# sparsemat/sprs

Measured on AMD Instinct MI355X. Metric: CSR SpMV GFLOP/s, higher is better.
Workload: dtype f64; 1 GPU; R-MAT 10M x 10M, ~32 nnz/row (Graph500 a,b,c,d=.57,.19,.19,.05; seed 1); rows=10000000, cols=10000000, nnz=321592231, index_bytes=8, indptr_bytes=8, partition=single GPU, first_spmv_plan=nnz tiles

## Files before the change

### sprs_amd/csrc/spmv_band_kernels.hpp

```cpp
#pragma once
#include "spmv_shared.hpp"

namespace sprs_hip {
namespace {

typedef uint32_t u32x4 __attribute__((ext_vector_type(4)));

constexpr int WT = 512;
constexpr int WPASS = WT / (WAVE * 2);
constexpr int EPL = WT / WAVE;
constexpr int HOT_THREADS = 1024;
constexpr int HOT_WAVES = HOT_THREADS / WAVE;
constexpr int CNT = 256;
constexpr uint32_t ROW_START = 0x8000u;
constexpr uint32_t ROW_START32 = 0x80000000u;
static_assert(WPASS == 4 && EPL == 8, "wave tile geometry");

struct BandPiece {
    const uint32_t *rowidx;
    const uint32_t *tile_row;
    double *out;
    uint64_t ent0;
    uint64_t nnz;
    uint32_t nr, ntiles;
    uint32_t x0;
    uint32_t to_y;
    uint32_t range0;
    uint32_t pad;
};

struct Seg {
    uint32_t piece, tile0, ntiles, range0, run, pad0, pad1, pad2;
};

struct alignas(64) HotSeg {
    uint64_t ent0, nnz;
    const uint32_t *tile_row;
    uint64_t out_off;
    uint32_t x0, tile0, ntiles, range0;
    uint32_t run, pad0, pad1, pad2;
};
static_assert(sizeof(HotSeg) == 64, "one scalar load");

struct ColdGroup {
    uint32_t first_block, first_piece, npieces;
};

#ifdef SPRS_HIP_EMU
#define SPRS_GLOBAL_AS
#define SPRS_HOT_WAVES_ATTR
#else
#define SPRS_GLOBAL_AS __attribute__((address_space(1)))
#define SPRS_HOT_WAVES_ATTR __attribute__((amdgpu_waves_per_eu(5, 5)))
#endif
struct PieceView {
    const SPRS_GLOBAL_AS uint32_t *rowidx, *tile_row;
    SPRS_GLOBAL_AS double *out;
    uint64_t ent0, nnz;
    uint32_t nr, ntiles, x0, to_y, range0;
    __device__ __forceinline__ PieceView(const BandPiece &p)
        : rowidx((const SPRS_GLOBAL_AS uint32_t *)p.rowidx), tile_row((const SPRS_GLOBAL_AS uint32_t *)p.tile_row),
          out((SPRS_GLOBAL_AS double *)p.out), ent0(p.ent0), nnz(p.nnz), nr(p.nr), ntiles(p.ntiles), x0(p.x0), to_y(p.to_y),
          range0(p.range0) {}
};

__device__ __forceinline__ uint32_t band_scan_incl_u32(uint32_t v, uint32_t lane) {
    (void)lane;
    int x = (int)v;
    x += __builtin_amdgcn_update_dpp(0, x, 0x111, 0xf, 0xf, true);
    x += __builtin_amdgcn_update_dpp(0, x, 0x112, 0xf, 0xf, true);
    x += __builtin_amdgcn_update_dpp(0, x, 0x114, 0xf, 0xf, true);
    x += __builtin_amdgcn_update_dpp(0, x, 0x118, 0xf, 0xf, true);
    x += __builtin_amdgcn_update_dpp(0, x, 0x142, 0xa, 0xf, false);
    x += __builtin_amdgcn_update_dpp(0, x, 0x143, 0xc, 0xf, false);
    return (uint32_t)x;
}

template <int CTRL, int ROW_MASK, bool BOUND>
__device__ __forceinline__ void band_seg_step(double &S, uint32_t &F) {
    const int lo = __builtin_amdgcn_update_dpp(0, __double2loint(S), CTRL, ROW_MASK, 0xf, BOUND);
    const int hi = __builtin_amdgcn_update_dpp(0, __double2hiint(S), CTRL, ROW_MASK, 0xf, BOUND);
    const uint32_t fs = (uint32_t)__builtin_amdgcn_update_dpp(0, (int)F, CTRL, ROW_MASK, 0xf, BOUND);
    const double vs = __hiloint2double(hi, lo);
    S = F ? S : vs + S;
    F |= fs;
}

__device__ __forceinline__ void band_seg_scan(double &S, uint32_t &F, uint32_t lane) {
    (void)lane;
    band_seg_step<0x111, 0xf, true>(S, F);
    band_seg_step<0x112, 0xf, true>(S, F);
    band_seg_step<0x114, 0xf, true>(S, F);
    band_seg_step<0x118, 0xf, true>(S, F);
    band_seg_step<0x142, 0xa, false>(S, F);
    band_seg_step<0x143, 0xc, false>(S, F);
}

__device__ __forceinline__ double band_lane_below(double S, uint32_t lane) {
    (void)lane;
    const int lo = __builtin_amdgcn_update_dpp(0, __double2loint(S), 0x138, 0xf, 0xf, true);
    const int hi = __builtin_amdgcn_update_dpp(0, __double2hiint(S), 0x138, 0xf, 0xf, true);
    return __hiloint2double(hi, lo);
}

__device__ __forceinline__ double band_read_lane63(double v) {
    const int lo = __builtin_amdgcn_readlane(__double2loint(v), WAVE - 1);
    const int hi = __builtin_amdgcn_readlane(__double2hiint(v), WAVE - 1);
    return __hiloint2double(hi, lo);
}

__device__ __forceinline__ void wave_lds_fence() {
    __builtin_amdgcn_fence(__ATOMIC_RELEASE, "wavefront");
    __builtin_amdgcn_wave_barrier();
    __builtin_amdgcn_fence(__ATOMIC_ACQUIRE, "wavefront");
}

constexpr int STG = 128;
constexpr uint32_t hot_lds_bytes(uint32_t xt_log2) { return ((1u << xt_log2) + (uint32_t)HOT_WAVES * 128u) * 8u; }

struct Pending {
    uint32_t cnt = 0;
    uint32_t row0 = 0;
    bool first_to_carry = false;
};

template <typename Out>
__device__ __forceinline__ void band_flush(Pending &pd, uint32_t lane, SPRS_GLOBAL_AS double *carry, const double *stage, Out out) {
    for (uint32_t j = lane; j < pd.cnt; j += WAVE) {
        const double v = stage[j];
        if (j == 0 && pd.first_to_carry) *carry = v;
        else out(pd.row0 + j, v);
    }
    wave_lds_fence();
    pd.cnt = 0;
}

template <bool DEFER, typename Out>
__device__ __forceinline__ void band_tile_sums(const double (&pr)[EPL], uint32_t fb, uint32_t lane, uint32_t R0, double &open, bool &mine,
                                               uint32_t &last, SPRS_GLOBAL_AS double *carry, double *stage, Pending &pd, Out out) {
    const uint32_t nfl = (uint32_t)__popc(fb);
    const uint32_t incl = band_scan_incl_u32(nfl, lane);
    const uint32_t prefix = incl - nfl;
    const uint32_t nf = (uint32_t)__builtin_amdgcn_readlane((int)incl, WAVE - 1);
    double ev[EPL];
    double run = 0.0, head = 0.0;
    uint32_t seen = 0;
#pragma unroll
    for (int q = 0; q < EPL; ++q) {
        ev[q] = run;
        if ((fb >> q) & 1u) {
            if (seen == 0) head = run;
            run = 0.0;
            ++seen;
        }
        run += pr[q];
    }
    double S = run;
    uint32_t F = seen ? 1u : 0u;
    band_seg_scan(S, F, lane);
    double before = band_lane_below(S, lane);
    if (prefix == 0) before = open + before;
    const double vhead = before + head;
    for (uint32_t lo = 0; lo < nf; lo += STG) {
#pragma unroll
        for (int q = 0; q < EPL; ++q) {
            if ((fb >> q) & 1u) {
                const uint32_t below = fb & ((1u << q) - 1u);
                const uint32_t o = prefix + (uint32_t)__popc(below) - lo;
                if (o < (uint32_t)STG) stage[o] = below ? ev[q] : vhead;
            }
        }
        wave_lds_fence();
        pd.cnt = nf - lo < (uint32_t)STG ? nf - lo : (uint32_t)STG;
        pd.row0 = R0 - 1u + lo;
        pd.first_to_carry = lo == 0 && !mine;
        if (!DEFER || lo + STG < nf) band_flush(pd, lane, carry, stage, out);
    }
    const double s63 = band_read_lane63(S);
    open = nf ? s63 : open + s63;
    if (nf) {
        mine = true;
        last = R0 + nf - 1;
    }
}

template <bool ACC, bool TOY>
__device__ __forceinline__ void band_cold_wave(const PieceView d, uint32_t r, uint32_t ct, const double *__restrict__ vals,
                                               const uint32_t *__restrict__ cid, const double *__restrict__ xp, double *__restrict__ y,
                                               double *__restrict__ carry, double *stage, uint32_t lane);

template <int XT_LOG2>
__global__ __launch_bounds__(HOT_THREADS) SPRS_HOT_WAVES_ATTR void band_hot_kernel(const HotSeg *__restrict__ hsegs,
                                                               const HotSeg *__restrict__ wg_first, const double *__restrict__ vals,
                                                               const uint16_t *__restrict__ cid, const double *__restrict__ xp,
                                                               double *__restrict__ partial, double *__restrict__ carry, uint32_t dbg,
                                                               unsigned long long *__restrict__ prof, uint32_t xcd_shares) {
    constexpr int XT = 1 << XT_LOG2;
    if constexpr (DEVTOOLS) {
        if (prof && threadIdx.x == 0) prof[3 * blockIdx.x] = (unsigned long long)wall_clock64();
    }
#ifdef SPRS_HIP_EMU
    static double lds[XT + HOT_WAVES * STG];
#else
    extern __shared__ __attribute__((aligned(16))) double lds[];
#endif
    double *xs = lds;
    const uint32_t tid = threadIdx.x, lane = tid & (WAVE - 1), wave = tid / WAVE;
    double *stage = lds + XT + wave * STG;
    uint32_t share = blockIdx.x;
    if (xcd_shares) {
        const uint32_t nq = gridDim.x >> 3, rem = gridDim.x & 7u, k = blockIdx.x & 7u;
        share = k * nq + (k < rem ? k : rem) + (blockIdx.x >> 3);
    }
    HotSeg nxt = wg_first[share];
    const uint32_t s0 = nxt.pad0, s1 = nxt.pad1;
    for (uint32_t s = s0; s < s1; ++s) {
        const HotSeg seg = nxt;
        if (s + 1 < s1) nxt = hsegs[s + 1];
        struct {
            const SPRS_GLOBAL_AS uint32_t *tile_row;
            SPRS_GLOBAL_AS double *out;
            uint64_t ent0, nnz;
            uint32_t x0;
        } d{(const SPRS_GLOBAL_AS uint32_t *)seg.tile_row, (SPRS_GLOBAL_AS double *)(partial + seg.out_off), seg.ent0, seg.nnz, seg.x0};
        if (s != s0) __syncthreads();
        {
            const dbl2 *src = (const dbl2 *)(xp + d.x0);
            dbl2 v[XT / (2 * HOT_THREADS)];
#pragma unroll
            for (int q = 0; q < XT / (2 * HOT_THREADS); ++q) v[q] = src[q * HOT_THREADS + tid];
#pragma unroll
            for (int q = 0; q < XT / (2 * HOT_THREADS); ++q) *(dbl2 *)&xs[2 * (q * HOT_THREADS + tid)] = v[q];
        }
        const uint32_t run = seg.run, n = seg.ntiles;
        dbl2 av[WPASS];
        u32x4 cw = {0u, 0u, 0u, 0u};
        uint32_t R0n = 0;
        auto request = [&](uint32_t w) {
            const uint64_t g = d.ent0 + (uint64_t)w * WT;
#pragma unroll
            for (int p = 0; p < WPASS; ++p) av[p] = __builtin_nontemporal_load((const dbl2 *)(vals + g + p * (WAVE * 2) + lane * 2));
            cw = __builtin_nontemporal_load((const u32x4 *)(cid + g + lane * EPL));
            R0n = d.tile_row[w];
        };
        uint32_t r = wave;
        uint32_t t = r * run;
        if (t < n) request(seg.tile0 + t);
        __syncthreads();
        if constexpr (DEVTOOLS) {
            if (prof && threadIdx.x == 0 && s == s0) prof[3 * blockIdx.x + 1] = (unsigned long long)wall_clock64();
        }
        double open = 0.0;
        bool mine = false;
        uint32_t last = 0;
        Pending pd;
        SPRS_GLOBAL_AS double *pd_slot = (SPRS_GLOBAL_AS double *)carry;
        while (t < n) {
            const uint32_t w = seg.tile0 + t;
            const uint64_t base = (uint64_t)w * WT;
            const uint32_t cnt = d.nnz - base < (uint64_t)WT ? (uint32_t)(d.nnz - base) : (uint32_t)WT;
            double pr[EPL], xv[EPL];
            uint32_t fb = 0;
#pragma unroll
            for (int p = 0; p < WPASS; ++p) {
                const uint32_t c2 = cw[p];
                xv[2 * p] = xs[c2 & (XT - 1)];
                xv[2 * p + 1] = xs[(c2 >> 16) & (XT - 1)];
                fb |= ((c2 >> 15) & 1u) << (2 * p);
                fb |= ((c2 >> 31) & 1u) << (2 * p + 1);
            }
#pragma unroll
            for (int p = 0; p < WPASS; ++p) {
                pr[2 * p] = av[p][0] * xv[2 * p];
                pr[2 * p + 1] = av[p][1] * xv[2 * p + 1];
            }
            if (cnt < (uint32_t)WT) {
#pragma unroll
                for (int q = 0; q < EPL; ++q) pr[q] = lane * EPL + q < cnt ? pr[q] : 0.0;
            }
            uint32_t R0 = R0n;
#ifndef SPRS_HIP_EMU
            asm volatile("" : "+v"(R0)::"memory");
#endif
            const uint32_t rend = (r + 1) * run < n ? (r + 1) * run : n;
            const bool range_ends = t + 1 >= rend;
            const uint32_t tn = range_ends ? (r + HOT_WAVES) * run : t + 1;
            SPRS_GLOBAL_AS double *cslot = (SPRS_GLOBAL_AS double *)carry + seg.range0 + r;
            auto out = [&](uint32_t row, double v) {
                if (DEVTOOLS && (dbg & 1u)) return;
                __builtin_nontemporal_store(v, &d.out[row]);

            };
            if (pd.cnt) band_flush(pd, lane, pd_slot, stage, out);
            if (tn < n) request(seg.tile0 + tn);
            if constexpr (DEVTOOLS) {
                if (dbg & 2u) fb &= 0x01u;
                if (dbg & 4u) fb = 0;
            }
            if (DEVTOOLS && (dbg & 8u)) {
                band_tile_sums<false>(pr, fb, lane, R0, open, mine, last, cslot, stage, pd, out);
            } else {
                band_tile_sums<true>(pr, fb, lane, R0, open, mine, last, cslot, stage, pd, out);
                pd_slot = cslot;
            }
            if (range_ends) {
                if (lane == 0) {
                    if (mine) d.out[last] = open;
                    else *cslot = open;
                }
                open = 0.0;
                mine = false;
                r += HOT_WAVES;
            }
            t = tn;
        }
        if (pd.cnt) band_flush(pd, lane, pd_slot, stage, [&](uint32_t row, double v) {
            if (DEVTOOLS && (dbg & 1u)) return;
            d.out[row] = v;
        });
    }
    if constexpr (DEVTOOLS) {
        if (prof) {
            __syncthreads();
            if (threadIdx.x == 0) prof[3 * blockIdx.x + 2] = (unsigned long long)wall_clock64();
        }
    }
}

struct ColdArgs {
    const BandPiece *pieces;
    const ColdGroup *groups;
    uint32_t ngroups;
    const double *vals;
    const uint32_t *cid;
    const double *xp;
    double *y, *carry;
    uint32_t block0, ct;
    uint32_t direct;
    BandPiece piece;
};

template <bool ACC, bool TOY>
__device__ __forceinline__ void band_cold_body(const ColdArgs &ca, uint32_t block, double (*stage_s)[STG]) {
    constexpr int WPB = CNT / WAVE;
    const BandPiece *__restrict__ pieces = ca.pieces;
    const ColdGroup *__restrict__ groups = ca.groups;
    const uint32_t ngroups = ca.ngroups, ct = ca.ct;
    const double *__restrict__ vals = ca.vals;
    const uint32_t *__restrict__ cid = ca.cid;
    const double *__restrict__ xp = ca.xp;
    double *__restrict__ y = ca.y;
    double *__restrict__ carry = ca.carry;
    const uint32_t tid = threadIdx.x, lane = tid & (WAVE - 1), wave = tid / WAVE;
    double *stage = stage_s[wave];
    const uint32_t bid = block + ca.block0;
    uint32_t r;
    BandPiece pc;
    if (ca.direct) {
        pc = ca.piece;
        r = block * WPB + wave;
    } else {
        uint32_t g = 0;
        while (g + 1 < ngroups && bid >= groups[g + 1].first_block) ++g;
        const ColdGroup cg = groups[g];
        const uint32_t lb = bid - cg.first_block;
        const uint32_t pi = cg.first_piece + (cg.npieces == 1 ? 0u : (lb & 7u));
        r = (cg.npieces == 1 ? lb : (lb >> 3)) * WPB + wave;
        pc = pieces[pi];
    }
    band_cold_wave<ACC, TOY>(PieceView(pc), r, ct, vals, cid, xp, y, carry, stage, lane);
}

template <bool ACC, bool TOY>
__device__ __forceinline__ void band_cold_wave(const PieceView d, uint32_t r, uint32_t ct, const double *__restrict__ vals,
                                               const uint32_t *__restrict__ cid, const double *__restrict__ xp, double *__restrict__ y,
                                               double *__restrict__ carry, double *stage, uint32_t lane) {
    const uint32_t t0 = r * ct;
    if (t0 >= d.ntiles) return;
    const uint32_t tend = t0 + ct < d.ntiles ? t0 + ct : d.ntiles;
    dbl2 av[WPASS];
    u32x4 lw[2];
    uint32_t R0n = 0;
    auto request = [&](uint32_t w) {
        const uint64_t gpos = d.ent0 + (uint64_t)w * WT;
#pragma unroll
        for (int p = 0; p < 2; ++p) lw[p] = __builtin_nontemporal_load((const u32x4 *)(cid + gpos + p * (WAVE * 4) + lane * 4));
#pragma unroll
        for (int p = 0; p < WPASS; ++p) av[p] = __builtin_nontemporal_load((const dbl2 *)(vals + gpos + p * (WAVE * 2) + lane * 2));
        R0n = d.tile_row[w];
    };
    request(t0);
    double open = 0.0;
    bool mine = false;
    uint32_t last = 0;
    SPRS_GLOBAL_AS double *cslot = (SPRS_GLOBAL_AS double *)carry + d.range0 + r;
    uint32_t yr_pre[4] = {0u, 0u, 0u, 0u}, yr_base = 0;
    auto emit_y = [&](uint32_t row, double v) {
        const uint32_t m = (row - yr_base) >> 6;
        uint32_t yr;
        if (TOY && m < 4u && ((row - yr_base) & 63u) == lane) yr = m == 0 ? yr_pre[0] : m == 1 ? yr_pre[1] : m == 2 ? yr_pre[2] : yr_pre[3];
        else yr = d.rowidx[row];
        if constexpr (ACC) y[yr] = y[yr] + v;
        else y[yr] = v;
    };
    auto emit_p = [&](uint32_t row, double v) { d.out[row] = v; };
    for (uint32_t w = t0; w < tend; ++w) {
        const uint64_t base = (uint64_t)w * WT;
        const uint32_t cnt = d.nnz - base < (uint64_t)WT ? (uint32_t)(d.nnz - base) : (uint32_t)WT;
        double xv[EPL];
        uint32_t fb = 0;
#pragma unroll
        for (int q = 0; q < EPL; ++q) {
            const uint32_t c = lw[q / 4][q % 4];
            xv[q] = xp[c & ~ROW_START32];
            fb |= (c >> 31) << q;
        }
        if constexpr (TOY) {
            yr_base = R0n - 1u;
#pragma unroll
            for (int m = 0; m < 4; ++m) {
                const uint32_t rr = yr_base + lane + 64u * (uint32_t)m;
                yr_pre[m] = d.rowidx[rr < d.nr ? rr : d.nr - 1u];
            }
        }
        double pr[EPL];
#pragma unroll
        for (int q = 0; q < EPL; ++q) pr[q] = av[q / 2][q % 2] * xv[q];
        if (cnt < (uint32_t)WT) {
#pragma unroll
            for (int q = 0; q < EPL; ++q) pr[q] = lane * EPL + q < cnt ? pr[q] : 0.0;
        }
        Pending pd;
        if constexpr (TOY) band_tile_sums<false>(pr, fb, lane, R0n, open, mine, last, cslot, stage, pd, emit_y);
        else band_tile_sums<false>(pr, fb, lane, R0n, open, mine, last, cslot, stage, pd, emit_p);
        if (w + 1 < tend) request(w + 1);
    }
    if (lane == 0) {
        if (!mine) *cslot = open;
        else if constexpr (TOY) emit_y(last, open);
        else emit_p(last, open);
    }
}

template <bool ACC, bool TOY>
__global__ __launch_bounds__(CNT, 8) void band_cold_kernel(ColdArgs ca) {
    __shared__ __attribute__((aligned(16))) double stage_s[CNT / WAVE][STG];
    band_cold_body<ACC, TOY>(ca, blockIdx.x, stage_s);
}

struct RangeRef {
    uint32_t piece, tile0;
    bool valid;
};

__device__ __forceinline__ RangeRef range_of(const Seg *__restrict__ segs, uint32_t nsegs, uint32_t i) {
    uint32_t lo = 0, hi = nsegs;
    while (hi - lo > 1) {
        const uint32_t mid = (lo + hi) >> 1;
        if (segs[mid].range0 <= i) lo = mid;
        else hi = mid;
    }
    const Seg sg = segs[lo];
    const uint32_t t = (i - sg.range0) * sg.run;
    return RangeRef{sg.piece, sg.tile0 + t, t < sg.ntiles};
}

__device__ __forceinline__ bool range_has_head(const BandPiece &d, uint32_t piece, uint32_t tile0, const uint16_t *__restrict__ cid_hot,
                                               const uint32_t *__restrict__ cid_cold, uint32_t nhot) {
    const uint64_t e = d.ent0 + (uint64_t)tile0 * WT;
    return piece < nhot ? !(cid_hot[e] & ROW_START) : !(cid_cold[e] & ROW_START32);
}

struct Spill {
    uint64_t dst;
    uint32_t first, n;
    uint32_t to_y, j;
};

struct RSpill {
    uint32_t j, first, n, pad;
};

__global__ __launch_bounds__(256) void bp_spill_kernel(const Seg *__restrict__ segs, uint32_t nsegs, uint32_t nranges,
                                                       const BandPiece *__restrict__ pieces, const uint64_t *__restrict__ pair_off,
                                                       uint32_t nhot, const uint16_t *__restrict__ cid_hot,
                                                       const uint32_t *__restrict__ cid_cold,
                                                       Spill *__restrict__ spills_y, Spill *__restrict__ spills_partial,
                                                       unsigned int *__restrict__ count) {
    const uint32_t i = blockIdx.x * blockDim.x + threadIdx.x;
    if (i >= nranges) return;
    const RangeRef rg = range_of(segs, nsegs, i);
    if (!rg.valid) return;
    const BandPiece d = pieces[rg.piece];
    if (!range_has_head(d, rg.piece, rg.tile0, cid_hot, cid_cold, nhot)) return;
    const uint32_t row = d.tile_row[rg.tile0] - 1;
    if (i > 0) {
        const RangeRef pj = range_of(segs, nsegs, i - 1);
        if (pj.valid && pj.piece == rg.piece && d.tile_row[pj.tile0] - 1 == row && range_has_head(d, pj.piece, pj.tile0, cid_hot, cid_cold, nhot))
            return;
    }
    uint32_t n = 1;
    for (uint32_t j = i + 1; j < nranges; ++j, ++n) {
        const RangeRef nj = range_of(segs, nsegs, j);
        if (!nj.valid || nj.piece != rg.piece || d.tile_row[nj.tile0] - 1 != row || !range_has_head(d, nj.piece, nj.tile0, cid_hot, cid_cold, nhot))
            break;
    }
    const bool first = d.to_y != 0;
    const unsigned int slot = atomicAdd(count + (first ? 0 : 1), 1u);
    (first ? spills_y : spills_partial)[slot] = Spill{d.to_y ? (uint64_t)d.rowidx[row] : pair_off[rg.piece] + row, i, n, d.to_y, d.rowidx[row]};
}

template <bool TO_Y>
__global__ __launch_bounds__(256) void band_carry_kernel(const Spill *__restrict__ spills, uint32_t nspills, const double *__restrict__ carry,
                                                         double *__restrict__ partial, double *__restrict__ y) {
    const uint32_t i = blockIdx.x * blockDim.x + threadIdx.x;
    if (i >= nspills) return;
    const Spill sp = spills[i];
    double *dst = (TO_Y ? y : partial) + sp.dst;
    double acc = *dst;
    for (uint32_t k = 0; k < sp.n; ++k) acc += carry[sp.first + k];
    *dst = acc;
}

template <bool CLEAR_Y>
__global__ __launch_bounds__(256) void band_gather_kernel(const double *__restrict__ x, const uint32_t *__restrict__ inv, uint32_t l0,
                                                          uint32_t l1, double *__restrict__ xp, double *__restrict__ y_zero, uint64_t rows) {
    const uint64_t t4 = ((uint64_t)blockIdx.x * blockDim.x + threadIdx.x) * 4;
    const uint64_t l = (uint64_t)l0 + t4;
    if (l + 4 <= (uint64_t)l1 && (l0 & 3u) == 0) {
        const u32x4 j = *(const u32x4 *)(inv + l);
        const double a0 = x[j[0]], a1 = x[j[1]], a2 = x[j[2]], a3 = x[j[3]];
        *(dbl2 *)(xp + l) = dbl2{a0, a1};
        *(dbl2 *)(xp + l + 2) = dbl2{a2, a3};
    } else {
        for (uint64_t q = l; q < (uint64_t)l1 && q < l + 4; ++q) xp[q] = x[inv[q]];
    }
    if (CLEAR_Y && y_zero) {
        if (t4 + 4 <= rows && ((uintptr_t)y_zero & 15) == 0) {
            *(dbl2 *)(y_zero + t4) = dbl2{0.0, 0.0};
            *(dbl2 *)(y_zero + t4 + 2) = dbl2{0.0, 0.0};
        } else {
            for (uint64_t r = t4; r < rows && r < t4 + 4; ++r) y_zero[r] = 0.0;
        }
    }
}

__global__ __launch_bounds__(256) void band_permute_kernel(const double *__restrict__ x, const uint32_t *__restrict__ perm,
                                                           uint64_t cols, double *__restrict__ xp, double *__restrict__ y_zero,
                                                           uint64_t rows, uint32_t first_label, uint32_t nref) {
    const uint64_t j = ((uint64_t)blockIdx.x * blockDim.x + threadIdx.x) * 4;
    const uint32_t span = nref - first_label;
    if (j + 4 <= cols && (((uintptr_t)x | (uintptr_t)perm) & 15) == 0) {
        const u32x4 l = *(const u32x4 *)(perm + j);
        const dbl2 a = *(const dbl2 *)(x + j), b = *(const dbl2 *)(x + j + 2);
        if (l[0] - first_label < span) xp[l[0]] = a[0];
        if (l[1] - first_label < span) xp[l[1]] = a[1];
        if (l[2] - first_label < span) xp[l[2]] = b[0];
        if (l[3] - first_label < span) xp[l[3]] = b[1];
    } else {
        for (uint64_t c = j; c < cols && c < j + 4; ++c) {
            const uint32_t l = perm[c];
            if (l - first_label < span) xp[l] = x[c];
        }
    }
    if (y_zero) {
        if (j + 4 <= rows && ((uintptr_t)y_zero & 15) == 0) {
            *(dbl2 *)(y_zero + j) = dbl2{0.0, 0.0};
            *(dbl2 *)(y_zero + j + 2) = dbl2{0.0, 0.0};
        } else {
            for (uint64_t r = j; r < rows && r < j + 4; ++r) y_zero[r] = 0.0;
        }
    }
}

constexpr int RU = 16;

__device__ __forceinline__ bool band_mask_bit(uint32_t m_lo, uint32_t m_hi, uint32_t lane) {
    (void)lane;
    return __builtin_amdgcn_inverse_ballot_w64(((unsigned long long)m_hi << 32) | m_lo);
}
__device__ __forceinline__ uint32_t band_mask_rank(uint32_t m_lo, uint32_t m_hi, uint32_t lane) {
    (void)lane;
    return __builtin_amdgcn_mbcnt_hi(m_hi, __builtin_amdgcn_mbcnt_lo(m_lo, 0u));
}

struct ReduceArgs {
    const double *partial;
    const unsigned long long *wmask;
    const uint32_t *wbase, *long_rows;
    const RSpill *rsp;
    const uint32_t *rsp_off;
    const double *carry;
    double *y;
    uint32_t n_long, np_pad, nwb;
};

template <bool ACC>
__device__ __forceinline__ void band_reduce_body(const ReduceArgs &ra, uint32_t block, uint32_t nblocks) {
    const double *__restrict__ partial = ra.partial;
    const unsigned long long *__restrict__ wmask = ra.wmask;
    const uint32_t *__restrict__ wbase = ra.wbase;
    const uint32_t *__restrict__ long_rows = ra.long_rows;
    double *__restrict__ y = ra.y;
    const uint32_t n_long = ra.n_long, np_pad = ra.np_pad, nwb = ra.nwb;
    const uint32_t lane = threadIdx.x & (WAVE - 1);
    const uint32_t wpb = blockDim.x / WAVE;
    const uint32_t xcd = block & 7u, inx = (block >> 3) * wpb + threadIdx.x / WAVE;
    const uint32_t per_xcd = (nwb + 7u) / 8u, waves_per_xcd = (nblocks >> 3) * wpb;
    for (uint32_t i = inx; i < per_xcd; i += waves_per_xcd) {
        const uint32_t wb = xcd * per_xcd + i;
        if (wb >= nwb) break;
        const uint64_t j = (uint64_t)wb * WAVE + lane;
        const uint64_t jc = j < n_long ? j : n_long - 1;
        const uint32_t r = long_rows[jc];
        uint32_t sb = 0, se = 0;
        if (ra.rsp_off) {
            sb = ra.rsp_off[wb];
            se = ra.rsp_off[wb + 1];
        }
        uint32_t h_jl = 0xFFFFFFFFu, h_first = 0, h_n = 0;
        double h_c = 0.0;
        if (sb + lane < se) {
            const RSpill rec = ra.rsp[sb + lane];
            h_jl = rec.j & (WAVE - 1);
            h_first = rec.first;
            h_n = rec.n;
            h_c = ra.carry[h_first];
        }
        double s = 0.0;
        const unsigned long long *mrow = wmask + (uint64_t)wb * np_pad;
        const uint32_t *brow = wbase + (uint64_t)wb * np_pad;
        unsigned long long mk_n = lane < np_pad ? mrow[lane] : 0ull;
        uint32_t bs_n = lane < np_pad ? brow[lane] : 0u;
        for (uint32_t k0 = 0; k0 < np_pad; k0 += WAVE) {
            const unsigned long long mk = mk_n;
            const uint32_t bs = bs_n;
            if (k0 + WAVE < np_pad) {
                const bool in = k0 + WAVE + lane < np_pad;
                mk_n = in ? mrow[k0 + WAVE + lane] : 0ull;
                bs_n = in ? brow[k0 + WAVE + lane] : 0u;
            }
            const uint32_t mk_lo = (uint32_t)mk, mk_hi = (uint32_t)(mk >> 32);
#pragma unroll
            for (int kk = 0; kk < WAVE; kk += RU) {
                if (k0 + kk >= np_pad) break;
                double v[RU];
#pragma unroll
                for (int u = 0; u < RU; ++u) {
                    const uint32_t m_lo = (uint32_t)__builtin_amdgcn_readlane((int)mk_lo, kk + u);
                    const uint32_t m_hi = (uint32_t)__builtin_amdgcn_readlane((int)mk_hi, kk + u);
                    const uint32_t b = (uint32_t)__builtin_amdgcn_readlane((int)bs, kk + u);
                    v[u] = band_mask_bit(m_lo, m_hi, lane) ? partial[b + band_mask_rank(m_lo, m_hi, lane)] : 0.0;
                }
#pragma unroll
                for (int u = 0; u < RU; ++u) s += v[u];
            }
        }
        for (uint32_t i0 = sb; i0 < se; i0 += WAVE) {
            if (i0 != sb) {
                h_jl = 0xFFFFFFFFu;
                h_n = 0;
                h_c = 0.0;
                if (i0 + lane < se) {
                    const RSpill rec = ra.rsp[i0 + lane];
                    h_jl = rec.j & (WAVE - 1);
                    h_first = rec.first;
                    h_n = rec.n;
                    h_c = ra.carry[h_first];
                }
            }
            for (uint32_t k = 1; k < h_n; ++k) h_c += ra.carry[h_first + k];
            const uint32_t cnt = se - i0 < (uint32_t)WAVE ? se - i0 : (uint32_t)WAVE;
            for (uint32_t t = 0; t < cnt; ++t) {
                const uint32_t tj = (uint32_t)__builtin_amdgcn_readlane((int)h_jl, (int)t);
                const int lo = __builtin_amdgcn_readlane(__double2loint(h_c), (int)t);
                const int hi = __builtin_amdgcn_readlane(__double2hiint(h_c), (int)t);
                if (lane == tj) s += __hiloint2double(hi, lo);
            }
        }
        if (j < n_long) {
            if constexpr (ACC) y[r] = y[r] + s;
            else y[r] = s;
        }
    }
}

template <bool ACC>
__global__ __launch_bounds__(256) void band_reduce_kernel(ReduceArgs ra) {
    band_reduce_body<ACC>(ra, blockIdx.x, gridDim.x);
}

template <bool ACC>
__global__ __launch_bounds__(CNT, 8) void band_tail_kernel(ReduceArgs ra, uint32_t reduce_blocks, ColdArgs ca) {
    __shared__ __attribute__((aligned(16))) double stage_s[CNT / WAVE][STG];
    if (blockIdx.x < reduce_blocks) band_reduce_body<ACC>(ra, blockIdx.x, reduce_blocks);
    else band_cold_body<ACC, true>(ca, blockIdx.x - reduce_blocks, stage_s);
}

}
}
```

Measured before the change: 628.0 GFLOP/s.

## Software-pipeline band reduce gathers in alternating half-groups with branchless clamped loads

Restructures the long-row reduce loop so that partial-sum gathers for one half-group of 8 window entries are issued while the previous half-group is being accumulated. Mask and base tables for the next 64-entry window are prefetched on the wrap. Loads are made unconditional: indices are clamped, and masked-out lanes read a valid address whose value is then dropped. Pointers are cast to the global address space, and carry loads are unrolled to a fixed 8 with clamping. This is meant to hide gather latency and remove divergent branches, at the cost of extra redundant loads and a hard cap of 8 carries per spill record.

```diff
diff --git a/sprs_amd/csrc/spmv_band_kernels.hpp b/sprs_amd/csrc/spmv_band_kernels.hpp
--- a/sprs_amd/csrc/spmv_band_kernels.hpp
+++ b/sprs_amd/csrc/spmv_band_kernels.hpp
@@ -574,6 +574,9 @@
 }
 
 constexpr int RU = 16;
+constexpr int RH = 8;
+constexpr int RC = 8;
+static_assert(RU == 2 * RH && WAVE % RU == 0, "the groups of a chunk alternate between the two halves of the window");
 
 __device__ __forceinline__ bool band_mask_bit(uint32_t m_lo, uint32_t m_hi, uint32_t lane) {
     (void)lane;
@@ -597,88 +600,137 @@
 
 template <bool ACC>
 __device__ __forceinline__ void band_reduce_body(const ReduceArgs &ra, uint32_t block, uint32_t nblocks) {
-    const double *__restrict__ partial = ra.partial;
-    const unsigned long long *__restrict__ wmask = ra.wmask;
-    const uint32_t *__restrict__ wbase = ra.wbase;
-    const uint32_t *__restrict__ long_rows = ra.long_rows;
+    const SPRS_GLOBAL_AS double *__restrict__ partial = (const SPRS_GLOBAL_AS double *)ra.partial;
+    const SPRS_GLOBAL_AS double *__restrict__ carry = (const SPRS_GLOBAL_AS double *)ra.carry;
+    const SPRS_GLOBAL_AS unsigned long long *__restrict__ wmask = (const SPRS_GLOBAL_AS unsigned long long *)ra.wmask;
+    const SPRS_GLOBAL_AS uint32_t *__restrict__ wbase = (const SPRS_GLOBAL_AS uint32_t *)ra.wbase;
+    const SPRS_GLOBAL_AS uint32_t *__restrict__ long_rows = (const SPRS_GLOBAL_AS uint32_t *)ra.long_rows;
+    typedef uint32_t u32x3 __attribute__((ext_vector_type(3)));
+    static_assert(sizeof(u32x3) == sizeof(RSpill), "a record per element");
+    const SPRS_GLOBAL_AS u32x3 *__restrict__ rsp = (const SPRS_GLOBAL_AS u32x3 *)ra.rsp;
     double *__restrict__ y = ra.y;
     const uint32_t n_long = ra.n_long, np_pad = ra.np_pad, nwb = ra.nwb;
     const uint32_t lane = threadIdx.x & (WAVE - 1);
+    if (np_pad == 0) return;
     const uint32_t wpb = blockDim.x / WAVE;
-    const uint32_t xcd = block & 7u, inx = (block >> 3) * wpb + threadIdx.x / WAVE;
+    const uint32_t wave = (uint32_t)__builtin_amdgcn_readfirstlane((int)(threadIdx.x / WAVE));
+    const uint32_t xcd = block & 7u, inx = (block >> 3) * wpb + wave;
     const uint32_t per_xcd = (nwb + 7u) / 8u, waves_per_xcd = (nblocks >> 3) * wpb;
     for (uint32_t i = inx; i < per_xcd; i += waves_per_xcd) {
         const uint32_t wb = xcd * per_xcd + i;
         if (wb >= nwb) break;
-        const uint64_t j = (uint64_t)wb * WAVE + lane;
-        const uint64_t jc = j < n_long ? j : n_long - 1;
-        const uint32_t r = long_rows[jc];
+        auto at = [&](const auto *base, uint32_t last, uint32_t l) {
+            typedef decltype(base) P;
+            const uint32_t off = (l < last ? l : last) * (uint32_t)sizeof(*base);
+            return *(P)((const SPRS_GLOBAL_AS char *)base + off);
+        };
+        const uint32_t row0 = wb * WAVE, rows = n_long - row0;
+        uint32_t r = at(long_rows + row0, rows - 1u, lane);
+        const SPRS_GLOBAL_AS unsigned long long *mrow = wmask + (uint64_t)wb * np_pad;
+        const SPRS_GLOBAL_AS uint32_t *brow = wbase + (uint64_t)wb * np_pad;
+        auto tables = [&](uint32_t k0, unsigned long long &mk, uint32_t &bs) {
+            mk = at(mrow + k0, np_pad - 1u - k0, lane);
+            bs = at(brow + k0, np_pad - 1u - k0, lane);
+        };
+        unsigned long long mk = 0ull, mk_n = 0ull;
+        uint32_t bs = 0u, bs_n = 0u;
+        tables(0u, mk, bs);
         uint32_t sb = 0, se = 0;
         if (ra.rsp_off) {
             sb = ra.rsp_off[wb];
             se = ra.rsp_off[wb + 1];
         }
-        uint32_t h_jl = 0xFFFFFFFFu, h_first = 0, h_n = 0;
-        double h_c = 0.0;
-        if (sb + lane < se) {
-            const RSpill rec = ra.rsp[sb + lane];
-            h_jl = rec.j & (WAVE - 1);
-            h_first = rec.first;
-            h_n = rec.n;
-            h_c = ra.carry[h_first];
-        }
+        RSpill rec{0u, 0u, 0u, 0u};
+        auto record = [&](uint32_t i0, uint32_t l) {
+            const u32x3 q = at(rsp + i0, se - 1u - i0, l);
+            rec = RSpill{q[0], q[1], q[2], 0u};
+        };
+        uint32_t l0 = lane;
+#ifndef SPRS_HIP_EMU
+        asm("" : "+v"(l0), "+v"(bs));
+#endif
+        if (se > sb) record(sb, l0);
+        double hc[RC];
+        auto carries = [&]() {
+            const uint32_t top = rec.n - 1u;
+#pragma unroll
+            for (int k = 0; k < RC; ++k) hc[k] = carry[rec.first + ((uint32_t)k < top ? (uint32_t)k : top)];
+        };
         double s = 0.0;
-        const unsigned long long *mrow = wmask + (uint64_t)wb * np_pad;
-        const uint32_t *brow = wbase + (uint64_t)wb * np_pad;
-        unsigned long long mk_n = lane < np_pad ? mrow[lane] : 0ull;
-        uint32_t bs_n = lane < np_pad ? brow[lane] : 0u;
-        for (uint32_t k0 = 0; k0 < np_pad; k0 += WAVE) {
-            const unsigned long long mk = mk_n;
-            const uint32_t bs = bs_n;
-            if (k0 + WAVE < np_pad) {
-                const bool in = k0 + WAVE + lane < np_pad;
-                mk_n = in ? mrow[k0 + WAVE + lane] : 0ull;
-                bs_n = in ? brow[k0 + WAVE + lane] : 0u;
-            }
-            const uint32_t mk_lo = (uint32_t)mk, mk_hi = (uint32_t)(mk >> 32);
-#pragma unroll
-            for (int kk = 0; kk < WAVE; kk += RU) {
-                if (k0 + kk >= np_pad) break;
-                double v[RU];
-#pragma unroll
-                for (int u = 0; u < RU; ++u) {
-                    const uint32_t m_lo = (uint32_t)__builtin_amdgcn_readlane((int)mk_lo, kk + u);
-                    const uint32_t m_hi = (uint32_t)__builtin_amdgcn_readlane((int)mk_hi, kk + u);
-                    const uint32_t b = (uint32_t)__builtin_amdgcn_readlane((int)bs, kk + u);
-                    v[u] = band_mask_bit(m_lo, m_hi, lane) ? partial[b + band_mask_rank(m_lo, m_hi, lane)] : 0.0;
+        auto request = [&](double (&v)[RH], unsigned long long gm, uint32_t gb, uint32_t kk) {
+            const uint32_t mk_lo = (uint32_t)gm, mk_hi = (uint32_t)(gm >> 32);
+#pragma unroll
+            for (int u = 0; u < RH; ++u) {
+                const uint32_t m_lo = (uint32_t)__builtin_amdgcn_readlane((int)mk_lo, (int)kk + u);
+                const uint32_t m_hi = (uint32_t)__builtin_amdgcn_readlane((int)mk_hi, (int)kk + u);
+                const uint32_t b = (uint32_t)__builtin_amdgcn_readlane((int)gb, (int)kk + u);
+                uint32_t rank = band_mask_bit(m_lo, m_hi, lane) ? band_mask_rank(m_lo, m_hi, lane) : 0u;
+#ifndef SPRS_HIP_EMU
+                asm("" : "+v"(rank));
+#endif
+                const SPRS_GLOBAL_AS char *run = (const SPRS_GLOBAL_AS char *)(partial + ((m_lo | m_hi) ? b : 0u));
+                v[u] = *(const SPRS_GLOBAL_AS double *)(run + (rank << 3));
+            }
+        };
+        auto add = [&](const double (&v)[RH], unsigned long long gm, uint32_t kk) {
+            const uint32_t mk_lo = (uint32_t)gm, mk_hi = (uint32_t)(gm >> 32);
+#pragma unroll
+            for (int u = 0; u < RH; ++u) {
+                const uint32_t m_lo = (uint32_t)__builtin_amdgcn_readlane((int)mk_lo, (int)kk + u);
+                const uint32_t m_hi = (uint32_t)__builtin_amdgcn_readlane((int)mk_hi, (int)kk + u);
+                s += band_mask_bit(m_lo, m_hi, lane) ? v[u] : 0.0;
+            }
+        };
+        {
+            double va[RH], vb[RH];
+            request(va, mk, bs, 0u);
+            if (WAVE < np_pad) tables(WAVE, mk_n, bs_n);
+            request(vb, mk, bs, (uint32_t)RH);
+            add(va, mk, 0u);
+            uint32_t k = 0;
+            for (; k + RU < np_pad; k += RU) {
+                const uint32_t kk = k & (WAVE - 1u);
+                const bool wrap = kk + RU == WAVE;
+                request(va, wrap ? mk_n : mk, wrap ? bs_n : bs, wrap ? 0u : kk + RU);
+                add(vb, mk, kk + RH);
+                if (wrap) {
+                    mk = mk_n;
+                    bs = bs_n;
+#ifndef SPRS_HIP_EMU
+                    asm("" : "+v"(mk), "+v"(bs), "+v"(s));
+#endif
+                    if (k + RU + WAVE < np_pad) tables(k + RU + WAVE, mk_n, bs_n);
                 }
-#pragma unroll
-                for (int u = 0; u < RU; ++u) s += v[u];
-            }
-        }
-        for (uint32_t i0 = sb; i0 < se; i0 += WAVE) {
-            if (i0 != sb) {
-                h_jl = 0xFFFFFFFFu;
-                h_n = 0;
-                h_c = 0.0;
-                if (i0 + lane < se) {
-                    const RSpill rec = ra.rsp[i0 + lane];
-                    h_jl = rec.j & (WAVE - 1);
-                    h_first = rec.first;
-                    h_n = rec.n;
-                    h_c = ra.carry[h_first];
+                const uint32_t kn = (k + RU) & (WAVE - 1u);
+                request(vb, mk, bs, kn + RH);
+                add(va, mk, kn);
+            }
+            const uint32_t kl = (k & (WAVE - 1u)) + RH;
+            if (se <= sb) {
+                add(vb, mk, kl);
+            } else {
+                carries();
+                add(vb, mk, kl);
+                for (uint32_t i0 = sb; i0 < se; i0 += WAVE) {
+                    if (i0 != sb) {
+                        record(i0, lane);
+                        carries();
+                    }
+                    double h_c = hc[0];
+#pragma unroll
+                    for (int q = 1; q < RC; ++q) h_c = (uint32_t)q < rec.n ? h_c + hc[q] : h_c;
+                    const uint32_t h_jl = rec.j & (WAVE - 1);
+                    const uint32_t cnt = se - i0 < (uint32_t)WAVE ? se - i0 : (uint32_t)WAVE;
+                    for (uint32_t t = 0; t < cnt; ++t) {
+                        const uint32_t tj = (uint32_t)__builtin_amdgcn_readlane((int)h_jl, (int)t);
+                        const int lo = __builtin_amdgcn_readlane(__double2loint(h_c), (int)t);
+                        const int hi = __builtin_amdgcn_readlane(__double2hiint(h_c), (int)t);
+                        if (lane == tj) s += __hiloint2double(hi, lo);
+                    }
                 }
             }
-            for (uint32_t k = 1; k < h_n; ++k) h_c += ra.carry[h_first + k];
-            const uint32_t cnt = se - i0 < (uint32_t)WAVE ? se - i0 : (uint32_t)WAVE;
-            for (uint32_t t = 0; t < cnt; ++t) {
-                const uint32_t tj = (uint32_t)__builtin_amdgcn_readlane((int)h_jl, (int)t);
-                const int lo = __builtin_amdgcn_readlane(__double2loint(h_c), (int)t);
-                const int hi = __builtin_amdgcn_readlane(__double2hiint(h_c), (int)t);
-                if (lane == tj) s += __hiloint2double(hi, lo);
-            }
-        }
-        if (j < n_long) {
+        }
+        if (lane < rows) {
             if constexpr (ACC) y[r] = y[r] + s;
             else y[r] = s;
         }
```

New measurement: 624.5 GFLOP/s. No clear change (-0.6%).
